# yeyupiaoling/VoiceprintRecognition-Pytorch

Hardware: AMD Instinct MI355X
Metric: utterances/sec embedded (3 s@16 kHz, Fbank-80, EcapaTdnn, bs=256) (higher is better)
Workload: dtype f16

## Files before the change

### voiceprintrecognition-pytorch_amd/csrc/conv1d.hip

```cpp
#include "common.h"

#include <type_traits>

namespace mv {

constexpr int CV_TC = 128;
constexpr int CV_TN = 128;
constexpr int CV_BK = 64;
constexpr int CV_THREADS = 256;
constexpr int CV_LDS_BYTES = 2 * (CV_TC + CV_TN) * CV_BK * 2;
constexpr int CV_LDS_BYTES_WIDE = 2 * (CV_TC + 160) * CV_BK * 2;
constexpr int CV_SMALL_NS = 4;
constexpr int CV_LDS_BYTES_SMALL = CV_SMALL_NS * (64 + 64) * CV_BK * 2;
constexpr int CV_TAIL_NS = 4;
constexpr int CV_LDS_BYTES_TAIL = CV_TAIL_NS * (CV_TC + CV_TN) * CV_BK * 2;
constexpr int CV_LDS_BYTES_BIG = 256 * (256 * 2 + 8);

struct ConvArgs {
    const void* x;
    const void* x2;
    int64_t ldx, ldx2;
    const float* in_scale;
    const float* in_shift;
    const half_t* w;
// ... 267 lines not shown
    for (int ni = 0; ni < NI; ++ni) {
        nl[ni] = wn * (NI * 16) + ni * 16 + (lane & 15);
        const int n = n0 + nl[ni];
        nb[ni] = 0;
        nt[ni] = 0;
        if ((a.row_bias != nullptr || a.gate != nullptr) && n < n_end) {
            nb[ni] = n / a.T_out;
            nt[ni] = n - nb[ni] * a.T_out;
        }
    }
    const float4v zero4 = float4v{0.0f, 0.0f, 0.0f, 0.0f};
    const float4v one4 = float4v{1.0f, 1.0f, 1.0f, 1.0f};
#pragma unroll
    for (int mi = 0; mi < MI; ++mi) {
        const int col = wc * (MI * 16) + mi * 16 + crow;
        const int co = co0 + col;
        const bool cok = co < a.cout;
        const float4v scale4 = (cok && a.scale != nullptr) ? *reinterpret_cast<const float4v*>(a.scale + co) : one4;
        const float4v shift4 = (cok && a.scale != nullptr) ? *reinterpret_cast<const float4v*>(a.shift + co) : zero4;
#pragma unroll
        for (int ni = 0; ni < NI; ++ni) {
            const bool ok = cok && n0 + nl[ni] < n_end;
            float4v v = acc[mi][ni];
            if (a.row_bias != nullptr && ok) v += *reinterpret_cast<const float4v*>(a.row_bias + (int64_t)nb[ni] * a.cout + co);
            v = act4(v, a.pre_act);
            v = v * scale4 + shift4;
            v = act4(v, a.post_act);
            if (a.gate != nullptr && ok)
                v *= *reinterpret_cast<const float4v*>(a.gate + ((int64_t)nb[ni] * a.gate_nseg + nt[ni] / a.gate_seg_len) * a.cout + co);
            half4v hv;
#pragma unroll
            for (int r = 0; r < 4; ++r) hv[r] = to_half_sat(v[r]);
            *reinterpret_cast<half4v*>(smem + nl[ni] * ROWB + col * 2) = hv;
        }
    }
    __syncthreads();
    constexpr int CPRW = TC / 8;
    half_t* y = reinterpret_cast<half_t*>(a.y);
    const bool vec_ok = (a.ldy % 8 == 0) && ((reinterpret_cast<uintptr_t>(a.y) & 15) == 0);
    for (int i = tid; i < TN * CPRW; i += NTHREADS) {
        const int row = i / CPRW, ch = i - row * CPRW;
        const int n = n0 + row;
        const int co = co0 + ch * 8;
        if (n >= n_end || co >= a.cout) continue;
        const char* src = smem + row * ROWB + ch * 16;
        half_t* dst = y + (int64_t)n * a.ldy + co;
        if (vec_ok && co + 8 <= a.cout) {
            const half4v lo = *reinterpret_cast<const half4v*>(src);
            const half4v hi = *reinterpret_cast<const half4v*>(src + 8);
            half8v o;
#pragma unroll
            for (int e = 0; e < 4; ++e) {
                o[e] = lo[e];
                o[e + 4] = hi[e];
            }
            *reinterpret_cast<half8v*>(dst) = o;
        } else {
            *reinterpret_cast<half4v*>(dst) = *reinterpret_cast<const half4v*>(src);
            if (co + 8 <= a.cout) *reinterpret_cast<half4v*>(dst + 4) = *reinterpret_cast<const half4v*>(src + 8);
        }
    }
}

__host__ __device__ __forceinline__ bool tile_of_index_geom(int n_tiles, int co_tiles, int bid, int& n_tile, int& co_tile) {
    const int nfull = n_tiles >> 3, rest = n_tiles & 7;
    const int main_ids = nfull * 8 * co_tiles;
    if (bid >= main_ids) {
        const int j = bid - main_ids;
        if (j >= rest * co_tiles) return false;
        co_tile = j / rest;
        n_tile = 8 * nfull + j - co_tile * rest;
        return true;
    }
    const int xcd = bid & 7;
    const int seq = bid >> 3;
    const int group = seq / (nfull * 8);
    const int base = group * 8;
    const int gw = co_tiles - base < 8 ? co_tiles - base : 8;
    const int idx = seq - nfull * base;
    const int n_local = idx / gw;
    co_tile = base + idx - n_local * gw;
    n_tile = xcd + 8 * n_local;
    return true;
}

__device__ __forceinline__ bool tile_of_index(const ConvArgs& a, int bid, int& n_tile, int& co_tile) {
    return tile_of_index_geom(a.n_tiles, a.co_tiles, bid, n_tile, co_tile);
}

__device__ __forceinline__ bool tile_of_block(const ConvArgs& a, int& n_tile, int& co_tile) {
    if (a.tail_nv > 0) {
        const int sub = (int)blockIdx.x / a.tail_nv, v = (int)blockIdx.x - sub * a.tail_nv;
        int nt = 0, ct = 0;
        if (!tile_of_index_geom(a.tail_n_tiles, a.tail_co_tiles, a.tail_vb0 + v, nt, ct)) return false;
        n_tile = a.tail_split * nt + (sub & (a.tail_split - 1));
        co_tile = a.tail_split * ct + sub / a.tail_split;
        return n_tile < a.n_tiles;
    }
    return tile_of_index(a, blockIdx.x, n_tile, co_tile);
}

struct InStats {
    float2v s1[4], s2[4];
};

template <int TN>
__device__ __forceinline__ void input_stats_accumulate(InStats& st, const char* xtile, int wave, int lane) {
    const int chunk = 2 * wave + (lane >> 5), g = lane & 31;
#pragma unroll
    for (int q = 0; q < 4; ++q) st.s1[q] = st.s2[q] = float2v{0.0f, 0.0f};
#pragma unroll
    for (int p = 0; p < TN / 32; ++p) {
        const int row = g + 32 * p;
        const half8v v = *reinterpret_cast<const half8v*>(xtile + lds_off(row, chunk));
#pragma unroll
        for (int q = 0; q < 4; ++q) {
            const float2v f = float2v{(float)v[2 * q], (float)v[2 * q + 1]};
            st.s1[q] += f;
            st.s2[q] = __builtin_elementwise_fma(f, f, st.s2[q]);
        }
    }
}

__device__ __forceinline__ void input_stats_reduce_store(const ConvArgs& a, const InStats& st, int c0, int n_tile, int wave, int lane) {
    const int chunk = 2 * wave + (lane >> 5), g = lane & 31;
    float r1[8], r2[8];
#pragma unroll
    for (int e = 0; e < 8; ++e) {
        float t1 = st.s1[e >> 1][e & 1], t2 = st.s2[e >> 1][e & 1];
        MV_OPAQUE(t1);
        MV_OPAQUE(t2);
        t1 = row16_sum(t1);
        t2 = row16_sum(t2);
        t1 += dpp_mov<DPP_ROW_BCAST15>(0.0f, t1);
        t2 += dpp_mov<DPP_ROW_BCAST15>(0.0f, t2);
        MV_OPAQUE(t1);
        MV_OPAQUE(t2);
        r1[e] = t1;
        r2[e] = t2;
    }
    const int c = c0 + chunk * 8;
    if (g == 16 && c < a.cin) {
        float* ps = a.in_sum + (int64_t)n_tile * a.cin + c;
        float* pq = a.in_sq + (int64_t)n_tile * a.cin + c;
        *reinterpret_cast<float4v*>(ps) = float4v{r1[0], r1[1], r1[2], r1[3]};
        *reinterpret_cast<float4v*>(ps + 4) = float4v{r1[4], r1[5], r1[6], r1[7]};
        *reinterpret_cast<float4v*>(pq) = float4v{r2[0], r2[1], r2[2], r2[3]};
        *reinterpret_cast<float4v*>(pq + 4) = float4v{r2[4], r2[5], r2[6], r2[7]};
    }
}

constexpr int CV_IN_STATS_GROUP = 4;
constexpr int CV_IN_STATS_BUF_BYTES = 2 * 2 * CV_IN_STATS_GROUP * CV_BK * 4;
__device__ __forceinline__ void input_stats_reduce_to_lds(const InStats& st, float* sbuf, int s, int wave, int lane) {
    const int chunk = 2 * wave + (lane >> 5), g = lane & 31;
    float r1[8], r2[8];
#pragma unroll
    for (int e = 0; e < 8; ++e) {
        float t1 = st.s1[e >> 1][e & 1], t2 = st.s2[e >> 1][e & 1];
        MV_OPAQUE(t1);
        MV_OPAQUE(t2);
        t1 = row16_sum(t1);
        t2 = row16_sum(t2);
        t1 += dpp_mov<DPP_ROW_BCAST15>(0.0f, t1);
        t2 += dpp_mov<DPP_ROW_BCAST15>(0.0f, t2);
        MV_OPAQUE(t1);
        MV_OPAQUE(t2);
        r1[e] = t1;
        r2[e] = t2;
    }
    if (g == 16) {
        float* b = sbuf + ((s / CV_IN_STATS_GROUP) & 1) * (2 * CV_IN_STATS_GROUP * CV_BK) + (s % CV_IN_STATS_GROUP) * CV_BK + chunk * 8;
        *reinterpret_cast<float4v*>(b) = float4v{r1[0], r1[1], r1[2], r1[3]};
        *reinterpret_cast<float4v*>(b + 4) = float4v{r1[4], r1[5], r1[6], r1[7]};
        *reinterpret_cast<float4v*>(b + CV_IN_STATS_GROUP * CV_BK) = float4v{r2[0], r2[1], r2[2], r2[3]};
        *reinterpret_cast<float4v*>(b + CV_IN_STATS_GROUP * CV_BK + 4) = float4v{r2[4], r2[5], r2[6], r2[7]};
    }
}
__device__ __forceinline__ void input_stats_flush(const ConvArgs& a, const float* sbuf, int s_last, int n_tile, int tid) {
    if (tid >= 2 * CV_IN_STATS_GROUP * CV_BK / 4) return;
    const int grp = s_last / CV_IN_STATS_GROUP;
    const int arr = tid / (CV_IN_STATS_GROUP * CV_BK / 4), idx = tid - arr * (CV_IN_STATS_GROUP * CV_BK / 4);
    const int sl = idx / (CV_BK / 4), c4 = (idx - sl * (CV_BK / 4)) * 4;
    const int s = grp * CV_IN_STATS_GROUP + sl, c = s * CV_BK + c4;
    if (s > s_last || c >= a.cin) return;
    const float4v v = *reinterpret_cast<const float4v*>(sbuf + (grp & 1) * (2 * CV_IN_STATS_GROUP * CV_BK) + arr * (CV_IN_STATS_GROUP * CV_BK) + sl * CV_BK + c4);
    float* dst = (arr ? a.in_sq : a.in_sum) + (int64_t)n_tile * a.cin + c;
    *reinterpret_cast<float4v*>(dst) = v;
}

template <int WC, int WN, int MI, int NI, bool INSTATS = false, int NS = 2>
__global__ __launch_bounds__(64 * WC * WN) void conv1d_glds_kernel(ConvArgs a) {
    constexpr int TC = WC * MI * 16, TN = WN * NI * 16, NW = WC * WN;
    constexpr int NTW = TC / 8 / NW, NTX = TN / 8 / NW;
    constexpr int STAGE_BYTES = (TC + TN) * CV_BK * 2;
    MV_DYN_SMEM(smem);
    int n_tile, co_tile;
    if (!tile_of_block(a, n_tile, co_tile)) return;
    const int tid = threadIdx.x;
    const int lane = tid & 63;
    const int wave = __builtin_amdgcn_readfirstlane(tid >> 6);
    const int wc = wave / WN, wn = wave % WN;
    int n0 = n_tile * TN, n_end = a.n_rows;
    if (a.per_utt) {
        const int ub = n_tile / a.tiles_per_utt;
        n0 = ub * a.T_out + (n_tile - ub * a.tiles_per_utt) * TN;
        n_end = (ub + 1) * a.T_out;
    }
    const int co0 = co_tile * TC;

    const int lrow = lane >> 3;
    const int kc = (lane & 7) ^ (lrow & 7);
    RowMap rm[NTX];
    const half_t* wsrc[NTW];
#pragma unroll
    for (int i = 0; i < NTX; ++i) {
        const int n = n0 + (wave * NTX + i) * 8 + lrow;
        if (n < n_end) {
            rm[i].b = n / a.T_out;
            rm[i].t = n - rm[i].b * a.T_out;
        } else {
            rm[i].b = -1;
            rm[i].t = 0;
        }
    }
#pragma unroll
    for (int i = 0; i < NTW; ++i) {
        const int co = co0 + (wave * NTW + i) * 8 + lrow;
        wsrc[i] = co < a.cout_pad ? a.w + (int64_t)co * a.k * a.cin_pad + kc * 8 : nullptr;
    }
    const half_t* xbase = reinterpret_cast<const half_t*>(a.x);
    if (a.grp_cout > 0) xbase += (int64_t)(co0 / a.grp_cout) * a.grp_cin;
    const half_t* zero = reinterpret_cast<const half_t*>(g_zero_page);
    const int kstages_per_tap = a.cin_pad / CV_BK;
    const int nstages = a.k * kstages_per_tap;

    const half_t* xrow[NTX];
    bool xok[NTX];
    int cur_tap = -1;
    const bool full_k = (a.cin % CV_BK) == 0;
    auto issue = [&](int s, int buf) {
        char* wt = smem + buf * STAGE_BYTES;
        char* xtile = wt + TC * CV_BK * 2;
        const int tap = s / kstages_per_tap;
        const int c0 = (s - tap * kstages_per_tap) * CV_BK;
        if (tap != cur_tap) {
            cur_tap = tap;
#pragma unroll
            for (int i = 0; i < NTX; ++i) {
                const int tin = input_time(a, rm[i].t, tap);
                xok[i] = rm[i].b >= 0 && tin >= 0;
                xrow[i] = xok[i] ? xbase + ((int64_t)rm[i].b * a.T_in + tin) * a.ldx + kc * 8 : zero;
            }
        }
        const bool ch_ok = full_k || c0 + kc * 8 < a.cin;
#pragma unroll
        for (int i = 0; i < NTX; ++i) glds16((xok[i] && ch_ok) ? xrow[i] + c0 : zero, xtile + (wave * NTX + i) * 1024);
        const int64_t woff = (int64_t)tap * a.cin_pad + c0;
#pragma unroll
        for (int i = 0; i < NTW; ++i) glds16(wsrc[i] != nullptr ? wsrc[i] + woff : zero, wt + (wave * NTW + i) * 1024);
    };

    float4v acc[MI][NI];
    conv_acc_init<MI, NI>(a, co0, wc, lane, acc);

    if constexpr (NS > 2) {
        static_assert(!INSTATS && NS <= 4, "the ring form has no fused statistics; its waits are written out for up to three stages in flight");
        constexpr int TPS = NTX + NTW;
        const unsigned smem_addr = lds_addr(smem);
        auto issue_ring = [&](int s) {
            const unsigned wt = smem_addr + (unsigned)((s % NS) * STAGE_BYTES);
            const unsigned xtile = wt + TC * CV_BK * 2;
            const int tap = s / kstages_per_tap;
            const int c0 = (s - tap * kstages_per_tap) * CV_BK;
            if (tap != cur_tap) {
                cur_tap = tap;
#pragma unroll
                for (int i = 0; i < NTX; ++i) {
                    const int tin = input_time(a, rm[i].t, tap);
                    xok[i] = rm[i].b >= 0 && tin >= 0;
                    xrow[i] = xok[i] ? xbase + ((int64_t)rm[i].b * a.T_in + tin) * a.ldx + kc * 8 : zero;
                }
            }
            const bool ch_ok = full_k || c0 + kc * 8 < a.cin;
#pragma unroll
            for (int i = 0; i < NTX; ++i) glds16_untracked((xok[i] && ch_ok) ? xrow[i] + c0 : zero, xtile + (unsigned)((wave * NTX + i) * 1024));
            const int64_t woff = (int64_t)tap * a.cin_pad + c0;
#pragma unroll
            for (int i = 0; i < NTW; ++i) glds16_untracked(wsrc[i] != nullptr ? wsrc[i] + woff : zero, wt + (unsigned)((wave * NTW + i) * 1024));
        };
        for (int s0 = 0; s0 < NS - 1 && s0 < nstages; ++s0) issue_ring(s0);
        for (int s = 0; s < nstages; ++s) {
            const int last = s + NS - 2 < nstages - 1 ? s + NS - 2 : nstages - 1;
            const int younger = last - s;
            if (younger >= 2) {
                wait_vm<2 * TPS>();
            } else if (younger == 1) {
                wait_vm<TPS>();
            } else {
                wait_vm<0>();
            }
            lds_barrier();
            if (s + NS - 1 < nstages) issue_ring(s + NS - 1);
            const char* wt = smem + (s % NS) * STAGE_BYTES;
            mma_stage<MI, NI>(wt, wt + TC * CV_BK * 2, wc, wn, lane, acc);
        }
        __syncthreads();
        if (a.y_f16 && a.sum_dst == nullptr) {
            conv_epilogue_staged<MI, NI, TC, TN, 64 * NW>(a, smem, n0, n_end, co0, wc, wn, lane, tid, acc);
        } else {
            conv_epilogue<MI, NI>(a, n0, n_end, co0, wc, wn, lane, acc);
        }
        return;
    }
    issue(0, 0);
    wait_all_loads();
    __syncthreads();
    InStats st;
    [[maybe_unused]] float* sbuf = reinterpret_cast<float*>(smem + NS * STAGE_BYTES);
    for (int s = 0; s < nstages; ++s) {
        const int buf = s & 1;
        if constexpr (INSTATS) {
            if (s >= 2 && (s - 1) % CV_IN_STATS_GROUP == 0) input_stats_flush(a, sbuf, s - 2, n_tile, tid);
        }
        if (s + 1 < nstages) issue(s + 1, buf ^ 1);
        const char* wt = smem + buf * STAGE_BYTES;
        if constexpr (INSTATS) {
            static_assert(NW == 4 && TN % 32 == 0, "input statistics: 256 threads, whole groups of 32 rows");
            mma_half_stage<MI, NI>(wt, wt + TC * CV_BK * 2, wc, wn, lane, 0, acc);
            if (s > 0) input_stats_reduce_to_lds(st, sbuf, s - 1, wave, lane);
            mma_half_stage<MI, NI>(wt, wt + TC * CV_BK * 2, wc, wn, lane, 1, acc);
            input_stats_accumulate<TN>(st, wt + TC * CV_BK * 2, wave, lane);
        } else {
            mma_stage<MI, NI>(wt, wt + TC * CV_BK * 2, wc, wn, lane, acc);
        }
        wait_all_loads();
        __syncthreads();
    }
    if constexpr (INSTATS) {
        input_stats_reduce_to_lds(st, sbuf, nstages - 1, wave, lane);
        __syncthreads();
        if (nstages >= 2 && (nstages - 1) % CV_IN_STATS_GROUP == 0) input_stats_flush(a, sbuf, nstages - 2, n_tile, tid);
        input_stats_flush(a, sbuf, nstages - 1, n_tile, tid);
    }
    if (a.y_f16 && a.sum_dst == nullptr) {
        conv_epilogue_staged<MI, NI, TC, TN, 64 * NW>(a, smem, n0, n_end, co0, wc, wn, lane, tid, acc);
    } else {
        conv_epilogue<MI, NI>(a, n0, n_end, co0, wc, wn, lane, acc);
    }
}

constexpr int CV_IN_STATS_TN_K = 160;
__global__ __launch_bounds__(CV_THREADS) void conv1d_in_stats_kernel(ConvArgs a) {
    constexpr int TN = CV_IN_STATS_TN_K, NW = CV_THREADS / 64, NTX = TN / 8 / NW;
    MV_DYN_SMEM(smem);
    const int n_tile = blockIdx.x, s = blockIdx.y;
    const int tid = threadIdx.x, lane = tid & 63;
    const int wave = __builtin_amdgcn_readfirstlane(tid >> 6);
    const int ub = n_tile / a.tiles_per_utt;
    const int n0 = ub * a.T_out + (n_tile - ub * a.tiles_per_utt) * TN, n_end = (ub + 1) * a.T_out;
    const int lrow = lane >> 3;
    const int kc = (lane & 7) ^ (lrow & 7);
    const int c0 = s * CV_BK;
    const half_t* xbase = reinterpret_cast<const half_t*>(a.x);
    const half_t* zero = reinterpret_cast<const half_t*>(g_zero_page);
    const bool ch_ok = c0 + kc * 8 < a.cin;
#pragma unroll
    for (int i = 0; i < NTX; ++i) {
        const int n = n0 + (wave * NTX + i) * 8 + lrow;
        const half_t* src = zero;
        if (n < n_end && ch_ok) {
            const int b = n / a.T_out, t = n - b * a.T_out;
            src = xbase + ((int64_t)b * a.T_in + t) * a.ldx + kc * 8 + c0;
        }
        glds16(src, smem + (wave * NTX + i) * 1024);
    }
    wait_all_loads();
    __syncthreads();
    InStats st;
    input_stats_accumulate<TN>(st, smem, wave, lane);
    input_stats_reduce_store(a, st, c0, n_tile, wave, lane);
}

constexpr int CVP_DMA_STEPS = 4;
constexpr int CVP_STAGE_BYTES = 65536;
constexpr int CVP_PARAM_OFF = 2 * CVP_STAGE_BYTES;
constexpr int CVP_PARAM_SLOT = 3 * 1024;
constexpr int CVP_LDS_BYTES = CVP_PARAM_OFF + 3 * CVP_PARAM_SLOT;

struct LdsParams {
    const char* par;
    int wc, q;
    __device__ __forceinline__ float4v at(int array, int mi) const {
        return *reinterpret_cast<const float4v*>(par + array * 1024 + (wc * 128 + mi * 16 + 4 * q) * 4);
    }
    __device__ __forceinline__ float4v bias4(int mi) const { return at(0, mi); }
    __device__ __forceinline__ float4v scale4(int mi) const { return at(1, mi); }
    __device__ __forceinline__ float4v shift4(int mi) const { return at(2, mi); }
};
struct LaneParams {
    float b[2], s[2], t[2];
    int qaddr;
    __device__ __forceinline__ float4v get(const float (&h)[2], int mi) const {
        const float src = h[mi >> 2];
        float4v r;
#pragma unroll
        for (int j = 0; j < 4; ++j) r[j] = lane_gather(src, qaddr + (mi & 3) * 64 + 4 * j);
        return r;
    }
    __device__ __forceinline__ float4v bias4(int mi) const { return get(b, mi); }
    __device__ __forceinline__ float4v scale4(int mi) const { return get(s, mi); }
    __device__ __forceinline__ float4v shift4(int mi) const { return get(t, mi); }
};

template <int STATS, bool HWSAT = false, class P>
__device__ __forceinline__ void persistent_epilogue(const ConvArgs& a, const P& par, int n0, int co0, int wc, int wn, int lane,
                                                    float4v (&acc)[8][4]) {
    static_assert(!HWSAT || STATS == 0, "the hardware-saturated form is the plain epilogue");
    const int r = lane & 15, q = lane >> 4;
    half_t* y = reinterpret_cast<half_t*>(a.y);
    const float lo_pre = a.pre_act == MV_ACT_RELU ? 0.0f : -INFINITY, lo_post = a.post_act == MV_ACT_RELU ? 0.0f : -65504.0f;
    const int ch_lane = (q & 1) * 16 + 4 * (q & ~1);
    const int first = n0 + wn * 64;
    const int split = STATS ? (first / a.T_out + 1) * a.T_out - first : 0;
    if constexpr (STATS == 0) {
        const bool wave_full = MV_UNIFORM(n0 + wn * 64 + 64 <= a.n_rows);
        auto halves = [&](auto FULL) __attribute__((always_inline)) {
#pragma unroll
        for (int h = 0; h < 2; ++h) {
            float4v sc[4], sh[4];
#pragma unroll
            for (int u = 0; u < 4; ++u) {
                sc[u] = par.scale4(4 * h + u);
                sh[u] = par.shift4(4 * h + u);
            }
            auto finish = [&](const float4v& c, int u) {
                float2v v0 = {max_raw(c[0], lo_pre), max_raw(c[1], lo_pre)};
                float2v v1 = {max_raw(c[2], lo_pre), max_raw(c[3], lo_pre)};
                v0 = v0 * float2v{sc[u][0], sc[u][1]} + float2v{sh[u][0], sh[u][1]};
                v1 = v1 * float2v{sc[u][2], sc[u][3]} + float2v{sh[u][2], sh[u][3]};
                half4v hv;
                if constexpr (HWSAT) {
                    hv[0] = half_hwsat(v0[0]);
                    hv[1] = half_hwsat(v0[1]);
                    hv[2] = half_hwsat(v1[0]);
                    hv[3] = half_hwsat(v1[1]);
                } else {
                    hv[0] = (half_t)clamp3(v0[0], lo_post, 65504.0f);
                    hv[1] = (half_t)clamp3(v0[1], lo_post, 65504.0f);
                    hv[2] = (half_t)clamp3(v1[0], lo_post, 65504.0f);
                    hv[3] = (half_t)clamp3(v1[1], lo_post, 65504.0f);
                }
                return hv;
            };
#pragma unroll
            for (int ni = 0; ni < 4; ++ni) {
                const int n = n0 + wn * 64 + ni * 16 + r;
                half_t* yrow = y + (int64_t)n * a.ldy + co0 + wc * 128 + ch_lane;
#pragma unroll
                for (int pp = 0; pp < 2; ++pp) {
                    const int p = 2 * h + pp;
                    const half4v ha = finish(acc[2 * p][ni], 2 * pp), hb = finish(acc[2 * p + 1][ni], 2 * pp + 1);
                    unsigned xa[2], xb[2];
                    __builtin_memcpy(xa, &ha, 8);
                    __builtin_memcpy(xb, &hb, 8);
                    row_swap_odd_even(xa[0], xb[0]);
                    row_swap_odd_even(xa[1], xb[1]);
                    const unsigned o[4] = {xa[0], xa[1], xb[0], xb[1]};
                    half8v ov;
                    __builtin_memcpy(&ov, o, 16);
                    if (decltype(FULL)::value || n < a.n_rows) *reinterpret_cast<half8v*>(yrow + p * 32) = ov;
                }
            }
        }
        };
        if (HWSAT && wave_full) {
            halves(std::true_type{});
        } else {
            halves(std::false_type{});
        }
        return;
    }
    const bool straddles = STATS && split < 64;
    float4v keep_sum[2], keep_sq[2];
    keep_sum[0] = keep_sum[1] = keep_sq[0] = keep_sq[1] = float4v{0.0f, 0.0f, 0.0f, 0.0f};
#pragma unroll
    for (int p = 0; p < 4; ++p) {
        float4v shift4[2], scale4[2];
        float4v s_sum[2][2], s_sq[2][2];
#pragma unroll
        for (int u = 0; u < 2; ++u) {
            shift4[u] = par.shift4(2 * p + u);
            scale4[u] = par.scale4(2 * p + u);
            s_sum[0][u] = s_sum[1][u] = s_sq[0][u] = s_sq[1][u] = float4v{0.0f, 0.0f, 0.0f, 0.0f};
        }
#pragma unroll
// ... 531 lines not shown
    int n_tile, co_tile;
    if (!tile_of_block(a, n_tile, co_tile)) return;
    const int tid = threadIdx.x;
    const int lane = tid & 63;
    const int wave = tid >> 6;
    const int wc = wave >> 1, wn = wave & 1;
    const int n0 = n_tile * CV_TN;
    const int co0 = co_tile * CV_TC;

    const int kc = tid & 7;
    const int lrow = tid >> 3;
    RowMap rm[4];
#pragma unroll
    for (int i = 0; i < 4; ++i) {
        const int n = n0 + lrow + 32 * i;
        if (n < a.n_rows) {
            rm[i].b = n / a.T_out;
            rm[i].t = n - rm[i].b * a.T_out;
        } else {
            rm[i].b = -1;
            rm[i].t = 0;
        }
    }
    const InT* xbase = reinterpret_cast<const InT*>(a.x);
    const InT* x2base = reinterpret_cast<const InT*>(a.x2);
    const InT* zero = reinterpret_cast<const InT*>(g_zero_page);
    const half_t* zero_h = reinterpret_cast<const half_t*>(g_zero_page);
    const int kstages_per_tap = a.cin_pad / CV_BK;
    const int nstages = a.k * kstages_per_tap;

    RawChunk<InT> xr[4], x2r[4];
    half8v wr[4];

    auto issue_loads = [&](int s) {
        const int tap = s / kstages_per_tap;
        const int c = (s - tap * kstages_per_tap) * CV_BK + kc * 8;
        const bool ch_ok = c < a.cin;
#pragma unroll
        for (int i = 0; i < 4; ++i) {
            const int tin = input_time(a, rm[i].t, tap);
            const bool ok = rm[i].b >= 0 && tin >= 0 && ch_ok;
            const int64_t row = (int64_t)rm[i].b * a.T_in + tin;
            load_raw(xr[i], ok ? xbase + row * a.ldx + c : zero);
            if (HAS_X2) load_raw(x2r[i], ok ? x2base + row * a.ldx2 + c : zero);
        }
#pragma unroll
        for (int i = 0; i < 4; ++i) {
            const int co = co0 + lrow + 32 * i;
            wr[i] = *MV_GLOBAL_PTR(half8v, co < a.cout_pad ? a.w + ((int64_t)co * a.k + tap) * a.cin_pad + c : zero_h);
        }
    };

    auto store_lds = [&](int s, int buf) {
        char* wt = smem + buf * ((CV_TC + CV_TN) * CV_BK * 2);
        char* xtile = wt + CV_TC * CV_BK * 2;
        const int tap = s / kstages_per_tap;
        const int c = (s - tap * kstages_per_tap) * CV_BK + kc * 8;
        float isc[8], ish[8];
        if (IN_AFFINE) {
            const int cc = c + 8 <= a.cin ? c : 0;
#pragma unroll
            for (int e = 0; e < 8; ++e) {
                isc[e] = a.in_scale[cc + e];
                ish[e] = a.in_shift[cc + e];
            }
        }
#pragma unroll
        for (int i = 0; i < 4; ++i) {
            const int row = lrow + 32 * i;
            half8v hv;
#pragma unroll
            for (int e = 0; e < 8; ++e) {
                float v = raw_get(xr[i], e);
                if (HAS_X2) v += raw_get(x2r[i], e);
                if (IN_AFFINE) v = fmaxf(__builtin_fmaf(v, isc[e], ish[e]), 0.0f);
                hv[e] = to_half_sat(v);
            }
            *reinterpret_cast<half8v*>(xtile + lds_off(row, kc)) = hv;
            *reinterpret_cast<half8v*>(wt + lds_off(row, kc)) = wr[i];
        }
    };

    float4v acc[4][4];
    conv_acc_init<4, 4>(a, co0, wc, lane, acc);

    issue_loads(0);
    store_lds(0, 0);
    __syncthreads();
    for (int s = 0; s < nstages; ++s) {
        const int buf = s & 1;
        if (s + 1 < nstages) issue_loads(s + 1);
        const char* wt = smem + buf * ((CV_TC + CV_TN) * CV_BK * 2);
        mma_stage<4, 4>(wt, wt + CV_TC * CV_BK * 2, wc, wn, lane, acc);
        if (s + 1 < nstages) store_lds(s + 1, buf ^ 1);
        __syncthreads();
    }
    conv_epilogue<4, 4>(a, n0, a.n_rows, co0, wc, wn, lane, acc);
}

__global__ void pack_conv_weight_kernel(const float* w, int cout, int cin, int k, int cout_pad, int cin_pad,
                                        half_t* out) {
    const int64_t total = (int64_t)cout_pad * k * cin_pad;
    for (int64_t i = (int64_t)blockIdx.x * blockDim.x + threadIdx.x; i < total; i += (int64_t)gridDim.x * blockDim.x) {
        const int ci = (int)(i % cin_pad);
        const int j = (int)((i / cin_pad) % k);
        const int co = (int)(i / ((int64_t)cin_pad * k));
        float v = 0.0f;
        if (co < cout && ci < cin) v = w[((int64_t)co * cin + ci) * k + j];
        out[i] = to_half_sat(v);
    }
}

__global__ void pack_conv_weight_grouped_kernel(const float* w, int cout, int cin, int k, int groups, int cout_pad, int cin_pad, half_t* out) {
    const int64_t total = (int64_t)cout_pad * k * cin_pad;
    const int cin_g = cin / groups, cout_g = cout / groups;
    for (int64_t i = (int64_t)blockIdx.x * blockDim.x + threadIdx.x; i < total; i += (int64_t)gridDim.x * blockDim.x) {
        const int ci = (int)(i % cin_pad);
        const int j = (int)((i / cin_pad) % k);
        const int co = (int)(i / ((int64_t)cin_pad * k));
        float v = 0.0f;
        if (co < cout && ci < cin && ci / cin_g == co / cout_g) v = w[((int64_t)co * cin_g + ci % cin_g) * k + j];
        out[i] = to_half_sat(v);
    }
}

bool conv1d_grouped_native(int cout, int cin, int k, int groups) {
    return groups > 1 && k == 1 && cin > 0 && cout > 0 && cin % groups == 0 && cout % groups == 0 && (cin / groups) % CV_BK == 0 &&
           (cout / groups) % 128 == 0;
}

int conv1d_cin_pad(int cin) { return (int)round_up(cin, CV_BK); }
int conv1d_cout_pad(int cout) { return (int)round_up(cout, 32); }


enum ConvKernel {
    CK_GLDS_128, CK_GLDS_64, CK_GLDS_128_TAIL, CK_GLDS_160, CK_GLDS_160_IN_STATS, CK_GLDS_256,
    CK_PERSIST_1X1, CK_PERSIST_1X1_SUM, CK_PERSIST_1X1_SUM_SQ,
    CK_PERSIST_TAPS,
    CK_RING, CK_RING_GROUPED,
    CK_MFMA_F32, CK_MFMA_X2, CK_MFMA_IN_AFFINE,
    CK_IN_STATS,
    CK_COUNT
};

struct ConvKernelRow {
    ConvKernel id;
    void (*fn)(ConvArgs);
    int threads, lds_bytes;
    int tile_rows, tile_ch;
    const char* name;
    const char* id_name;
};

template <int WC, int WN, int MI, int NI, bool INSTATS = false, int NS = 2>
constexpr ConvKernelRow glds_row(ConvKernel id, int lds_bytes, const char* name, const char* id_name) {
    return {id, conv1d_glds_kernel<WC, WN, MI, NI, INSTATS, NS>, 64 * WC * WN, lds_bytes, WN * NI * 16, WC * MI * 16, name, id_name};
}
#define MV_GLDS_ROW(id, lds_bytes, ...) glds_row<__VA_ARGS__>(id, lds_bytes, "conv1d_glds_kernel<" #__VA_ARGS__ ">", #id)
#define MV_CONV_ROW(id, threads, lds_bytes, tile_rows, tile_ch, ...) {id, __VA_ARGS__, threads, lds_bytes, tile_rows, tile_ch, #__VA_ARGS__, #id}
constexpr ConvKernelRow CONV_KERNELS[CK_COUNT] = {
    MV_GLDS_ROW(CK_GLDS_128, CV_LDS_BYTES, 2, 2, 4, 4),
    MV_GLDS_ROW(CK_GLDS_64, CV_LDS_BYTES_SMALL, 2, 2, 2, 2, false, CV_SMALL_NS),
    MV_GLDS_ROW(CK_GLDS_128_TAIL, CV_LDS_BYTES_TAIL, 4, 2, 2, 4, false, CV_TAIL_NS),
    MV_GLDS_ROW(CK_GLDS_160, CV_LDS_BYTES_WIDE, 2, 2, 4, 5),
    MV_GLDS_ROW(CK_GLDS_160_IN_STATS, CV_LDS_BYTES_WIDE + CV_IN_STATS_BUF_BYTES, 2, 2, 4, 5, true),
    MV_GLDS_ROW(CK_GLDS_256, CV_LDS_BYTES_BIG, 2, 4, 8, 4),
    MV_CONV_ROW(CK_PERSIST_1X1, 512, CVP_LDS_BYTES, 256, 256, conv1d_glds_persistent_kernel<true, 0>),
    MV_CONV_ROW(CK_PERSIST_1X1_SUM, 512, CVP_LDS_BYTES, 256, 256, conv1d_glds_persistent_kernel<true, 1>),
    MV_CONV_ROW(CK_PERSIST_1X1_SUM_SQ, 512, CVP_LDS_BYTES, 256, 256, conv1d_glds_persistent_kernel<true, 2>),
    MV_CONV_ROW(CK_PERSIST_TAPS, 512, CVP_LDS_BYTES, 256, 256, conv1d_glds_persistent_kernel<false, 0>),
    MV_CONV_ROW(CK_RING, 512, CVR_LDS_BYTES, 256, 256, conv1d_ring_persistent_kernel),
    MV_CONV_ROW(CK_RING_GROUPED, 512, CVR_LDS_BYTES, 256, 256, conv1d_ring_grouped_kernel),
    MV_CONV_ROW(CK_MFMA_F32, CV_THREADS, CV_LDS_BYTES, CV_TN, CV_TC, conv1d_mfma_kernel<float, false, false>),
    MV_CONV_ROW(CK_MFMA_X2, CV_THREADS, CV_LDS_BYTES, CV_TN, CV_TC, conv1d_mfma_kernel<half_t, true, false>),
    MV_CONV_ROW(CK_MFMA_IN_AFFINE, CV_THREADS, CV_LDS_BYTES, CV_TN, CV_TC, conv1d_mfma_kernel<half_t, false, true>),
    MV_CONV_ROW(CK_IN_STATS, CV_THREADS, CV_IN_STATS_TN * CV_BK * 2, CV_IN_STATS_TN, CV_BK, conv1d_in_stats_kernel),
};
#undef MV_GLDS_ROW
#undef MV_CONV_ROW
constexpr bool conv_kernels_in_enum_order(int i = 0) { return i == CK_COUNT || (CONV_KERNELS[i].id == i && conv_kernels_in_enum_order(i + 1)); }
static_assert(conv_kernels_in_enum_order(), "CONV_KERNELS has one row per ConvKernel, in the enum's order");


static int persistent_blocks(const MvConv1dDesc& d, int cus) { return (int)round_up(d.persist_blocks_hint > 0 ? d.persist_blocks_hint : cus, 8); }

static MvConv1dDesc one_group(const MvConv1dDesc& d_in, int groups) {
    MvConv1dDesc d = d_in;
    if (groups > 1) d.cin = d_in.cin / groups;
    return d;
}

static int conv1d_check(const MvConv1dDesc& d_in, int groups) {
    MV_REQUIRE(groups >= 1, "conv1d: groups must be positive");
    if (groups > 1) {
        MV_REQUIRE(conv1d_grouped_native(d_in.cout, d_in.cin, d_in.k, groups),
                   "conv1d: this grouped layer has no native form (1x1, cin / groups a multiple of 64, cout / groups a multiple of 128); "
                   "run its block-diagonal expansion (mv_conv1d_pack_weight_grouped) through the dense form");
        MV_REQUIRE(d_in.x_dtype == MV_DT_F16 && d_in.x2 == nullptr && d_in.in_scale == nullptr && d_in.stat_sum == nullptr &&
                       d_in.stat_sq == nullptr && d_in.in_stat_sum == nullptr && d_in.in_stat_sq == nullptr,
                   "conv1d: a grouped layer takes fp16 x without a second input, input affine or fused statistics");
        MV_REQUIRE(d_in.ldx >= d_in.cin, "conv1d: a grouped layer needs ldx >= cin (every group's slice of x)");
    }
    const MvConv1dDesc d = one_group(d_in, groups);
    MV_REQUIRE(d.x != nullptr && d.w_packed != nullptr && d.y != nullptr, "conv1d: null tensor");
    MV_REQUIRE(d.B > 0 && d.T_in > 0 && d.T_out > 0 && d.cin > 0 && d.cout > 0 && d.k > 0, "conv1d: bad geometry");
    MV_REQUIRE(d.dilation >= 1 && d.stride >= 1 && d.pad >= 0, "conv1d: bad dilation/stride/pad");
    MV_REQUIRE((int64_t)(d.T_out - 1) * d.stride - d.pad + (int64_t)(d.k - 1) * d.dilation < d.T_in + d.pad,
               "conv1d: T_out reaches beyond the padded input");
    if (d.pad_mode == MV_PAD_REFLECT) MV_REQUIRE(d.pad < d.T_in, "conv1d: reflect padding needs pad < T_in");
    MV_REQUIRE(d.x_dtype == MV_DT_F16 || d.x_dtype == MV_DT_F32, "conv1d: x dtype");
    MV_REQUIRE(d.y_dtype == MV_DT_F16 || d.y_dtype == MV_DT_F32, "conv1d: y dtype");
    MV_REQUIRE(d.pad_mode == MV_PAD_ZERO || d.pad_mode == MV_PAD_REFLECT, "conv1d: padding mode");
    MV_REQUIRE(d.pre_act >= MV_ACT_NONE && d.pre_act <= MV_ACT_SIGMOID && d.post_act >= MV_ACT_NONE && d.post_act <= MV_ACT_SIGMOID, "conv1d: activation code");
    MV_REQUIRE(d.ldx > 0 && d.ldy > 0 && (d.x2 == nullptr || d.ldx2 > 0) && (d.sum_dst == nullptr || (d.ld_add > 0 && d.ld_sum > 0)),
               "conv1d: leading dimensions must be positive");
    MV_REQUIRE((d.in_scale == nullptr) == (d.in_shift == nullptr), "conv1d: in_scale/in_shift go together");
    MV_REQUIRE((d.scale == nullptr) == (d.shift == nullptr), "conv1d: scale/shift go together");
    const int xalign = d.x_dtype == MV_DT_F16 ? 8 : 4;
    MV_REQUIRE(d.cin % 8 == 0, "conv1d: input channels must be a multiple of 8");
    MV_REQUIRE(d.cout % 4 == 0, "conv1d: output channels must be a multiple of 4");
    for (const float* p : {d.bias, d.row_bias, d.scale, d.shift, d.gate})
        MV_REQUIRE((reinterpret_cast<uintptr_t>(p) & 15) == 0, "conv1d: per-channel parameter arrays must be 16-byte aligned");
    MV_REQUIRE(d.ldx % xalign == 0 && (reinterpret_cast<uintptr_t>(d.x) & 15) == 0, "conv1d: x must be 16-byte aligned per row");
    if (d.x2 != nullptr)
        MV_REQUIRE(d.ldx2 % xalign == 0 && (reinterpret_cast<uintptr_t>(d.x2) & 15) == 0, "conv1d: x2 alignment");
    const int yalign_bytes = d.y_dtype == MV_DT_F16 ? 8 : 16;
    MV_REQUIRE(d.ldy % 4 == 0 && (reinterpret_cast<uintptr_t>(d.y) & (yalign_bytes - 1)) == 0, "conv1d: y alignment");
    if (d.gate != nullptr) MV_REQUIRE(d.gate_seg_len > 0, "conv1d: gate needs a segment length");
    if (d.in_scale != nullptr) MV_REQUIRE(d.pad == 0, "conv1d: the pre-activation on load is only defined for unpadded (1x1) convs");
    MV_REQUIRE((d.add_src == nullptr) == (d.sum_dst == nullptr), "conv1d: add_src/sum_dst go together");
    if (d.sum_dst != nullptr)
        MV_REQUIRE(d.ld_add % 4 == 0 && d.ld_sum % 4 == 0 && (reinterpret_cast<uintptr_t>(d.add_src) & 7) == 0 &&
                       (reinterpret_cast<uintptr_t>(d.sum_dst) & 7) == 0,
                   "conv1d: second output alignment");
    MV_REQUIRE((int64_t)d.B * d.T_out < ((int64_t)1 << 31) - CV_TN, "conv1d: too many rows for 32-bit indexing");
    MV_REQUIRE((reinterpret_cast<uintptr_t>(d.clock_probe) & 7) == 0, "conv1d: clock_probe must be 8-byte aligned");
    MV_REQUIRE((d.in_stat_sum == nullptr) == (d.in_stat_sq == nullptr), "conv1d: in_stat_sum / in_stat_sq go together");
    if (d.stat_sq != nullptr) MV_REQUIRE(d.stat_sum != nullptr, "conv1d: stat_sq needs stat_sum");
    MV_REQUIRE(d.tile == 0 || d.tile == 64 || d.tile == 128 || d.tile == 160 || d.tile == 256, "conv1d: tile must be 0 (auto), 64, 128, 160 or 256");
    return MV_OK;
}

struct ConvPlan {
    ConvKernel kernel = CK_GLDS_128, tail_kernel = CK_GLDS_64;
    int n_tiles = 0, co_tiles = 0;
    int grid = 0;
    int per_utt = 0, tiles_per_utt = 1;
    bool in_stats_first = false;
    int in_stats_tiles_per_utt = 0, in_stats_grid_x = 0, in_stats_grid_y = 0;
    int tail_vb0 = 0, tail_nv = 0, tail_split = 0;
    double tail_work = 0.0;
    int prof_class = MV_PROF_CONV1D;
    double work = 0.0;
};

static int conv1d_plan(const MvConv1dDesc& d, int groups, int cus, int blocks, ConvPlan* plan) {
    ConvPlan p;
    const int grp_cout = groups > 1 ? d.cout / groups : 0;
    const int n_rows = d.B * d.T_out, cin_pad = conv1d_cin_pad(d.cin);
    const int stats = d.stat_sum == nullptr ? 0 : (d.stat_sq == nullptr ? 1 : 2);
    const bool f16 = d.x_dtype == MV_DT_F16, has_x2 = d.x2 != nullptr, in_aff = d.in_scale != nullptr;
    const bool direct = f16 && !has_x2 && !in_aff;

    if (d.in_stat_sum != nullptr && direct && d.k == 1 && d.stride == 1 && d.pad == 0 && d.T_in == d.T_out && d.cout <= CV_TC && d.tile == 0 && d.cin % 8 == 0 &&
        (reinterpret_cast<uintptr_t>(d.in_stat_sum) & 15) == 0 && (reinterpret_cast<uintptr_t>(d.in_stat_sq) & 15) == 0 &&
        (int64_t)d.B * ceil_div(d.T_out, CV_IN_STATS_TN) * 2 <= (int64_t)cus && d.B <= 16384) {
        p.in_stats_first = true;
        p.in_stats_tiles_per_utt = (int)ceil_div(d.T_out, CV_IN_STATS_TN);
        p.in_stats_grid_x = d.B * p.in_stats_tiles_per_utt;
        p.in_stats_grid_y = cin_pad / CV_BK;
    }
    const bool in_stats = d.in_stat_sum != nullptr && !p.in_stats_first;

    const bool big_ok = f16 && !has_x2 && !in_aff && d.cout % 256 == 0 && grp_cout % 256 == 0;
    if (d.tile == 256) MV_REQUIRE(big_ok, "conv1d: 256-wide tiles need the plain fp16 path and cout % 256 == 0");
    const bool big = !in_stats && big_ok && d.tile != 128 && d.tile != 64 && d.tile != 160 &&
                     (d.tile == 256 || (int64_t)ceil_div(n_rows, 256) * (d.cout / 256) * 8 >= (int64_t)cus * 5);
    const bool plain = big && d.y_dtype == MV_DT_F16 && d.sum_dst == nullptr && d.row_bias == nullptr && d.gate == nullptr &&
                       d.ldy % 8 == 0 && (reinterpret_cast<uintptr_t>(d.y) & 15) == 0 &&
                       (d.pre_act == MV_ACT_NONE || d.pre_act == MV_ACT_RELU) &&
                       (d.post_act == MV_ACT_NONE || d.post_act == MV_ACT_RELU) &&
                       (int64_t)d.k * cin_pad >= 2 * CV_BK;
    const bool simple = d.k == 1 && d.cin % CV_BK == 0;
    const bool dense_rows = simple && d.stride == 1 && d.pad == 0 && d.T_in == d.T_out &&
                            (int64_t)n_rows * d.ldx * 2 < ((int64_t)1 << 32) && (int64_t)d.cout * cin_pad * 2 < ((int64_t)1 << 32);
    const bool ring = plain && stats == 0 && dense_rows && d.post_act == MV_ACT_NONE;
    const bool persist = ring || (plain && grp_cout == 0);

    bool wide = false;
    if (direct && !big) {
        if (d.tile == 160 || in_stats) {
            wide = true;
        } else if (d.tile == 0) {
            const int64_t slots = 2 * (int64_t)cus, cot = ceil_div(d.cout, CV_TC);
            const int64_t cost128 = ceil_div(ceil_div(n_rows, 128) * cot, slots) * 128;
            const int64_t cost160 = ceil_div(ceil_div(n_rows, 160) * cot, slots) * 160;
            wide = cost160 < cost128;
        }
    }
    if (d.tile == 160) MV_REQUIRE(direct && !big, "conv1d: the 160-row tile belongs to the plain fp16 path");
    const bool small = direct && !big && !wide && d.cout >= 64 &&
                       (d.tile == 64 || (d.tile == 0 && ceil_div(n_rows, CV_TN) * ceil_div(d.cout, CV_TC) * 2 <= (int64_t)cus));
    if (stats)
        MV_REQUIRE(persist && d.k == 1 && d.cin % CV_BK == 0 && d.T_out >= 64,
                   "conv1d: fused time statistics need the persistent 1x1 kernel (fp16 in/out, cout % 256 == 0, cin % 64 == 0, "
                   "plain bias / ReLU / affine epilogue, T_out >= 64)");
    if (in_stats) {
        MV_REQUIRE(direct && wide && d.k == 1 && d.stride == 1 && d.pad == 0 && d.T_in == d.T_out && d.cout <= CV_TC && d.tile != 128 &&
                       d.tile != 256 && (reinterpret_cast<uintptr_t>(d.in_stat_sum) & 15) == 0 && (reinterpret_cast<uintptr_t>(d.in_stat_sq) & 15) == 0,
                   "conv1d: fused input statistics need the direct fp16 1x1 path with the 160-row tile (stride 1, no padding, cout <= 128)");
        p.per_utt = 1;
        p.tiles_per_utt = (int)ceil_div(d.T_out, CV_IN_STATS_TN);
    }

    if (ring) {
        p.kernel = grp_cout > 0 ? CK_RING_GROUPED : CK_RING;
    } else if (persist) {
        p.kernel = stats == 2 ? CK_PERSIST_1X1_SUM_SQ : (stats == 1 ? CK_PERSIST_1X1_SUM : (simple ? CK_PERSIST_1X1 : CK_PERSIST_TAPS));
// ... 248 lines not shown
```

Measured before the change: 77870.

## Move fused input statistics in wide conv kernel onto dedicated extra waves

The wide 160-row conv kernel with fused input statistics now launches four extra waves that only compute per-channel sum and sum-of-squares from the staged input tiles, while the original four waves do just the MFMA loop. It also specializes the load issue path for the 1x1 statistics case by dropping tap and row-map lookups. The goal is to take the statistics arithmetic off the matrix-multiply critical path. In exchange the block doubles its thread count, which can cut occupancy, and the statistics waves must keep up through the shared barriers.

Result: no change. 77900, median of 2 (+0.0%).

```diff
diff --git a/voiceprintrecognition-pytorch_amd/csrc/conv1d.hip b/voiceprintrecognition-pytorch_amd/csrc/conv1d.hip
--- a/voiceprintrecognition-pytorch_amd/csrc/conv1d.hip
+++ b/voiceprintrecognition-pytorch_amd/csrc/conv1d.hip
@@ -443,6 +443,10 @@
 
 constexpr int CV_IN_STATS_GROUP = 4;
 constexpr int CV_IN_STATS_BUF_BYTES = 2 * 2 * CV_IN_STATS_GROUP * CV_BK * 4;
+constexpr int CV_WIDE_STATS_NS = 2;
+constexpr int CV_WIDE_STATS_WAVES = 4;
+constexpr bool CV_WIDE_STATS_RING = false;
+constexpr int CV_LDS_BYTES_WIDE_STATS = CV_WIDE_STATS_NS * (CV_TC + 160) * CV_BK * 2 + CV_IN_STATS_BUF_BYTES;
 __device__ __forceinline__ void input_stats_reduce_to_lds(const InStats& st, float* sbuf, int s, int wave, int lane) {
     const int chunk = 2 * wave + (lane >> 5), g = lane & 31;
     float r1[8], r2[8];
@@ -480,9 +484,34 @@
     *reinterpret_cast<float4v*>(dst) = v;
 }
 
-template <int WC, int WN, int MI, int NI, bool INSTATS = false, int NS = 2>
-__global__ __launch_bounds__(64 * WC * WN) void conv1d_glds_kernel(ConvArgs a) {
+template <int TN, int TC, int NS, int SW, bool RING>
+__device__ __forceinline__ void input_stats_waves(const ConvArgs& a, char* smem, int nstages, int n_tile, int swave, int lane, bool staged_epilogue) {
+    static_assert(SW == 2 || SW == 4, "two or four statistics waves walk the four waves' (chunk, half) pairs");
+    constexpr int STAGE_BYTES = (TC + TN) * CV_BK * 2, PER = 4 / SW;
+    float* sbuf = reinterpret_cast<float*>(smem + NS * STAGE_BYTES);
+    const int stid = swave * 64 + lane;
+    if constexpr (!RING) __syncthreads();
+    for (int s = 0; s < nstages; ++s) {
+        if constexpr (RING) lds_barrier();
+        if (s >= CV_IN_STATS_GROUP && s % CV_IN_STATS_GROUP == 0) input_stats_flush(a, sbuf, s - 1, n_tile, stid);
+        const char* xtile = smem + (s % NS) * STAGE_BYTES + TC * CV_BK * 2;
+#pragma unroll
+        for (int i = 0; i < PER; ++i) {
+            InStats st;
+            input_stats_accumulate<TN>(st, xtile, swave * PER + i, lane);
+            input_stats_reduce_to_lds(st, sbuf, s, swave * PER + i, lane);
+        }
+        if constexpr (!RING) __syncthreads();
+    }
+    if constexpr (RING) __syncthreads();
+    input_stats_flush(a, sbuf, nstages - 1, n_tile, stid);
+    if (staged_epilogue) __syncthreads();
+}
+
+template <int WC, int WN, int MI, int NI, bool INSTATS = false, int NS = 2, int SW = 0, bool RING = (NS > 2)>
+__global__ __launch_bounds__(64 * (WC * WN + SW)) void conv1d_glds_kernel(ConvArgs a) {
     constexpr int TC = WC * MI * 16, TN = WN * NI * 16, NW = WC * WN;
+    static_assert(INSTATS == (SW > 0) && (NS > 2 ? RING : true), "the fused statistics run on waves of their own; more than two stages are a ring");
     constexpr int NTW = TC / 8 / NW, NTX = TN / 8 / NW;
     constexpr int STAGE_BYTES = (TC + TN) * CV_BK * 2;
     MV_DYN_SMEM(smem);
@@ -499,6 +528,15 @@
         n_end = (ub + 1) * a.T_out;
     }
     const int co0 = co_tile * TC;
+    const int kstages_per_tap = a.cin_pad / CV_BK;
+    const int nstages = a.k * kstages_per_tap;
+    if constexpr (INSTATS) {
+        static_assert(NW == 4 && TN % 32 == 0, "input statistics: the (chunk, half) pairs of four waves, whole groups of 32 rows");
+        if (wave >= NW) {
+            input_stats_waves<TN, TC, NS, SW, RING>(a, smem, nstages, n_tile, wave - NW, lane, a.y_f16 && a.sum_dst == nullptr);
+            return;
+        }
+    }
 
     const int lrow = lane >> 3;
     const int kc = (lane & 7) ^ (lrow & 7);
@@ -523,8 +561,6 @@
     const half_t* xbase = reinterpret_cast<const half_t*>(a.x);
     if (a.grp_cout > 0) xbase += (int64_t)(co0 / a.grp_cout) * a.grp_cin;
     const half_t* zero = reinterpret_cast<const half_t*>(g_zero_page);
-    const int kstages_per_tap = a.cin_pad / CV_BK;
-    const int nstages = a.k * kstages_per_tap;
 
     const half_t* xrow[NTX];
     bool xok[NTX];
@@ -533,6 +569,19 @@
     auto issue = [&](int s, int buf) {
         char* wt = smem + buf * STAGE_BYTES;
         char* xtile = wt + TC * CV_BK * 2;
+        if constexpr (INSTATS) {
+            const int c0 = s * CV_BK;
+            const bool ch_ok = full_k || c0 + kc * 8 < a.cin;
+            const int r0 = n0 + wave * NTX * 8 + lrow;
+            const half_t* xp = xbase + (int64_t)r0 * a.ldx + kc * 8 + c0;
+#pragma unroll
+            for (int i = 0; i < NTX; ++i) glds16((r0 + i * 8 < n_end && ch_ok) ? xp + (int64_t)i * 8 * a.ldx : zero, xtile + (wave * NTX + i) * 1024);
+            const int w0 = co0 + wave * NTW * 8 + lrow;
+            const half_t* wp = a.w + (int64_t)w0 * a.cin_pad + kc * 8 + c0;
+#pragma unroll
+            for (int i = 0; i < NTW; ++i) glds16(w0 + i * 8 < a.cout_pad ? wp + (int64_t)i * 8 * a.cin_pad : zero, wt + (wave * NTW + i) * 1024);
+            return;
+        }
         const int tap = s / kstages_per_tap;
         const int c0 = (s - tap * kstages_per_tap) * CV_BK;
         if (tap != cur_tap) {
@@ -555,8 +604,8 @@
     float4v acc[MI][NI];
     conv_acc_init<MI, NI>(a, co0, wc, lane, acc);
 
-    if constexpr (NS > 2) {
-        static_assert(!INSTATS && NS <= 4, "the ring form has no fused statistics; its waits are written out for up to three stages in flight");
+    if constexpr (RING) {
+        static_assert(NS <= 4, "the ring's waits are written out for up to three stages in flight");
         constexpr int TPS = NTX + NTW;
         const unsigned smem_addr = lds_addr(smem);
         auto issue_ring = [&](int s) {
@@ -607,32 +656,13 @@
     issue(0, 0);
     wait_all_loads();
     __syncthreads();
-    InStats st;
-    [[maybe_unused]] float* sbuf = reinterpret_cast<float*>(smem + NS * STAGE_BYTES);
     for (int s = 0; s < nstages; ++s) {
         const int buf = s & 1;
-        if constexpr (INSTATS) {
-            if (s >= 2 && (s - 1) % CV_IN_STATS_GROUP == 0) input_stats_flush(a, sbuf, s - 2, n_tile, tid);
-        }
         if (s + 1 < nstages) issue(s + 1, buf ^ 1);
         const char* wt = smem + buf * STAGE_BYTES;
-        if constexpr (INSTATS) {
-            static_assert(NW == 4 && TN % 32 == 0, "input statistics: 256 threads, whole groups of 32 rows");
-            mma_half_stage<MI, NI>(wt, wt + TC * CV_BK * 2, wc, wn, lane, 0, acc);
-            if (s > 0) input_stats_reduce_to_lds(st, sbuf, s - 1, wave, lane);
-            mma_half_stage<MI, NI>(wt, wt + TC * CV_BK * 2, wc, wn, lane, 1, acc);
-            input_stats_accumulate<TN>(st, wt + TC * CV_BK * 2, wave, lane);
-        } else {
-            mma_stage<MI, NI>(wt, wt + TC * CV_BK * 2, wc, wn, lane, acc);
-        }
+        mma_stage<MI, NI>(wt, wt + TC * CV_BK * 2, wc, wn, lane, acc);
         wait_all_loads();
         __syncthreads();
-    }
-    if constexpr (INSTATS) {
-        input_stats_reduce_to_lds(st, sbuf, nstages - 1, wave, lane);
-        __syncthreads();
-        if (nstages >= 2 && (nstages - 1) % CV_IN_STATS_GROUP == 0) input_stats_flush(a, sbuf, nstages - 2, n_tile, tid);
-        input_stats_flush(a, sbuf, nstages - 1, n_tile, tid);
     }
     if (a.y_f16 && a.sum_dst == nullptr) {
         conv_epilogue_staged<MI, NI, TC, TN, 64 * NW>(a, smem, n0, n_end, co0, wc, wn, lane, tid, acc);
@@ -1470,9 +1500,9 @@
     const char* id_name;
 };
 
-template <int WC, int WN, int MI, int NI, bool INSTATS = false, int NS = 2>
+template <int WC, int WN, int MI, int NI, bool INSTATS = false, int NS = 2, int SW = 0, bool RING = (NS > 2)>
 constexpr ConvKernelRow glds_row(ConvKernel id, int lds_bytes, const char* name, const char* id_name) {
-    return {id, conv1d_glds_kernel<WC, WN, MI, NI, INSTATS, NS>, 64 * WC * WN, lds_bytes, WN * NI * 16, WC * MI * 16, name, id_name};
+    return {id, conv1d_glds_kernel<WC, WN, MI, NI, INSTATS, NS, SW, RING>, 64 * (WC * WN + SW), lds_bytes, WN * NI * 16, WC * MI * 16, name, id_name};
 }
 #define MV_GLDS_ROW(id, lds_bytes, ...) glds_row<__VA_ARGS__>(id, lds_bytes, "conv1d_glds_kernel<" #__VA_ARGS__ ">", #id)
 #define MV_CONV_ROW(id, threads, lds_bytes, tile_rows, tile_ch, ...) {id, __VA_ARGS__, threads, lds_bytes, tile_rows, tile_ch, #__VA_ARGS__, #id}
@@ -1481,7 +1511,7 @@
     MV_GLDS_ROW(CK_GLDS_64, CV_LDS_BYTES_SMALL, 2, 2, 2, 2, false, CV_SMALL_NS),
     MV_GLDS_ROW(CK_GLDS_128_TAIL, CV_LDS_BYTES_TAIL, 4, 2, 2, 4, false, CV_TAIL_NS),
     MV_GLDS_ROW(CK_GLDS_160, CV_LDS_BYTES_WIDE, 2, 2, 4, 5),
-    MV_GLDS_ROW(CK_GLDS_160_IN_STATS, CV_LDS_BYTES_WIDE + CV_IN_STATS_BUF_BYTES, 2, 2, 4, 5, true),
+    MV_GLDS_ROW(CK_GLDS_160_IN_STATS, CV_LDS_BYTES_WIDE_STATS, 2, 2, 4, 5, true, CV_WIDE_STATS_NS, CV_WIDE_STATS_WAVES, CV_WIDE_STATS_RING),
     MV_GLDS_ROW(CK_GLDS_256, CV_LDS_BYTES_BIG, 2, 4, 8, 4),
     MV_CONV_ROW(CK_PERSIST_1X1, 512, CVP_LDS_BYTES, 256, 256, conv1d_glds_persistent_kernel<true, 0>),
     MV_CONV_ROW(CK_PERSIST_1X1_SUM, 512, CVP_LDS_BYTES, 256, 256, conv1d_glds_persistent_kernel<true, 1>),
```
